# zouyuoz/SVS-UNet-PyTorch

Hardware: AMD Instinct MI355X
Metric: spectrogram-tiles/sec (512x128) U-Net fwd+bwd (L1 train step incl. Adam) (higher is better)
Workload: dtype f32; 1 GPU; train.py L1-loss step, 512x128 tiles, batch 64 per GPU; global_batch=64, parallelism=dp1, mode=train

## Files before the change

### svs_unet_pytorch_amd/csrc/common.h

```cpp
#pragma once
#include <hip/hip_runtime.h>
#include <stdint.h>
#include <stdio.h>
#include <string>
#include <type_traits>

#include "../../include/svs_hip.h"

typedef float f32x4 __attribute__((ext_vector_type(4)));

void svs_set_error(const char* fmt, ...);

#define SVS_REQUIRE(cond, ...)                 \
  do {                                         \
    if (!(cond)) {                             \
      svs_set_error(__VA_ARGS__);              \
      return SVS_ERR_INVALID;                  \
    }                                          \
  } while (0)

#define SVS_CHECK_LAUNCH(name)                                                     \
  do {                                                                             \
    hipError_t e_ = hipGetLastError();                                             \
    if (e_ != hipSuccess) {                                                        \
// ... 4 lines not shown

#define SVS_HIP(call)                                                              \
  do {                                                                             \
    hipError_t e_ = (call);                                                        \
    if (e_ != hipSuccess) {                                                        \
      svs_set_error("%s failed: %s", #call, hipGetErrorString(e_));                \
      return (int)e_;                                                              \
    }                                                                              \
  } while (0)

static inline bool svs_aligned16(const void* p) { return (((uintptr_t)p) & 15u) == 0; }
static inline int svs_cdiv(long a, long b) { return (int)((a + b - 1) / b); }
static inline size_t svs_align_up(size_t x, size_t a) { return (x + a - 1) / a * a; }

enum SvsTune {
  SVS_TUNE_CONV_CFG, SVS_TUNE_CONV_KSPLIT, SVS_TUNE_CONV_WINDOW, SVS_TUNE_CONV_SKIP, SVS_TUNE_SKIP_REDUCE,
  SVS_TUNE_WGRAD_CFG, SVS_TUNE_WGRAD_KSPLIT, SVS_TUNE_WGRAD_SKIP, SVS_TUNE_WGRAD_WINDOW, SVS_TUNE_TRAIN_UNFUSED,
  SVS_TUNE_TRAIN_ONE_STREAM, SVS_TUNE_MFMA_SPLIT, SVS_TUNE_CONV_C1_TILED, SVS_TUNE_BF16_CFG, SVS_TUNE_BF16_KSPLIT,
  SVS_TUNE_BN_INLINE, SVS_TUNE_CONV_GWINDOW, SVS_TUNE_COUNT
};
long svs_tune(int key);
static inline bool svs_tune_on(int key) { return svs_tune(key) >= 0; }
static inline bool svs_tune_flag(int key) { return svs_tune(key) > 0; }

static inline int svs_conv_out(int n) { return (n + 1) / 2; }

__device__ __forceinline__ float svs_wave_sum(float v) {
#pragma unroll
  for (int o = 32; o > 0; o >>= 1) v += __shfl_xor(v, o, 64);
  return v;
}

template <int N_, int I_ = 0, class F>
__device__ __forceinline__ void svs_static_for(F&& f) {
  if constexpr (I_ < N_) {
    f(std::integral_constant<int, I_>{});
    svs_static_for<N_, I_ + 1>(f);
  }
}

template <int R>
__device__ __forceinline__ float svs_quad_bcast(float x) {
  return __builtin_bit_cast(float, __builtin_amdgcn_update_dpp(0, __builtin_bit_cast(int, x), R * 0x55, 0xf, 0xf, true));
}

__device__ __forceinline__ int swz(int row, int chunk) { return chunk ^ ((row >> 1) & 3); }

__host__ __device__ __forceinline__ uint32_t svs_mix32(uint32_t x) {
  x ^= x >> 16; x *= 0x7FEB352Du; x ^= x >> 15; x *= 0x846CA68Bu; x ^= x >> 16;
  return x;
}
__host__ __device__ __forceinline__ uint32_t svs_u32(uint32_t seed, uint64_t idx) {
  uint32_t lo = (uint32_t)idx, hi = (uint32_t)(idx >> 32);
// ... 5 lines not shown
```

### svs_unet_pytorch_amd/csrc/elementwise.hip

```cpp
#include "unet_desc.h"

static inline int red_blocks(long P, int C) {
  long nb = (P * C) / 4096;
  if (nb > 1024) nb = 1024;
  if (nb < 1) nb = 1;
  return (int)nb;
}

struct RedPlan { int sw, nslab, lp, rows; long ppr; };
static RedPlan red_plan(long P, int C) {
  RedPlan r;
  r.sw = C < 32 ? C : 32;
  r.nslab = C / r.sw;
  r.lp = r.sw / 4;
  long nb = (P * C) / 4096;
  if (nb > 512) nb = 512;
  long rows = nb / r.nslab;
  if (rows < 1) rows = 1;
  r.ppr = (P + rows - 1) / rows;
  r.rows = (int)((P + r.ppr - 1) / r.ppr);
  return r;
}
static inline int red_rows(long P, int C) { return red_plan(P, C).rows; }

// ... 230 lines not shown
      if (row == 0) {
        if (dbeta) dbeta[c0 + t] = (float)s;
        if (dgamma) dgamma[c0 + t] = (float)sx;
      }
    }
    __syncthreads();
    k4 = *(const f32x4*)(p.gamma + c) * inv4;
    c1 = *(const f32x4*)&fin[0][l * 4];
    c2 = *(const f32x4*)&fin[1][l * 4];
  } else {
    k4 = *(const f32x4*)(coef + c);
    c1 = *(const f32x4*)(coef + p.C + c);
    c2 = *(const f32x4*)(coef + 2 * p.C + c);
  }
  const long p0 = (long)row * p.ppr;
  long p1 = p0 + p.ppr;
  if (p1 > p.P) p1 = p.P;
  f32x4 acc = {0.f, 0.f, 0.f, 0.f};
#pragma unroll 4
  for (long pix = p0 + pr; pix < p1; pix += PPB) {
    const f32x4 x = *(const f32x4*)(p.raw + pix * p.ldr + c);
    f32x4 dz = *(const f32x4*)(p.dy + pix * p.lddy + c);
    if (p.drop) dz *= *(const f32x4*)(p.drop + (long)((unsigned)pix / (unsigned)p.pps) * p.C + c);
    const f32x4 xm = x - mean4;
    const f32x4 z = xm * k4 + beta4;
#pragma unroll
    for (int k = 0; k < 4; ++k) dz[k] = z[k] > 0.f ? dz[k] : dz[k] * p.slope;
    const f32x4 r = k4 * (dz - c1 - (xm * inv4) * c2);
    *(f32x4*)(d_raw + pix * p.C + c) = r;
    acc += r;
  }
  if (partial) {
    red[t] = acc;
    __syncthreads();
    if (t < p.lp) {
      f32x4 a = red[t];
      for (int j = 1; j < PPB; ++j) a += red[j * p.lp + t];
      *(f32x4*)(partial + (long)row * 2 * p.C + c) = a;
    }
  }
}

static int check_bn(const char* who, const float* raw, long ldr, long P, int C) {
  SVS_REQUIRE(raw, "%s: null pointer", who);
  SVS_REQUIRE(C >= 4 && C % 4 == 0 && C <= 1024 && (256 % (C / 4) == 0 || (C / 4) % 256 == 0), "%s: unsupported C=%d", who, C);
  SVS_REQUIRE(P > 0 && P < (1L << 31) && ldr >= C && ldr % 4 == 0 && svs_aligned16(raw), "%s: bad view", who);
  return SVS_OK;
}

static int grid_for(long total) {
  long g = (total + 255) / 256;
// ... 64 lines not shown
}

extern "C" int svs_bn_act_apply(const float* raw, int64_t ldr, int64_t P, int C, int64_t pixels_per_sample,
                                const float* gamma, const float* beta, const float* save_mean, const float* save_invstd,
                                float slope, const float* drop, float* y, int64_t ldy, hipStream_t stream) {
  int rc = check_bn("svs_bn_act_apply", raw, ldr, P, C);
  if (rc) return rc;
  SVS_REQUIRE(y && ldy >= C && ldy % 4 == 0 && svs_aligned16(y), "svs_bn_act_apply: bad output view");
  BnCtx p{}; p.raw = raw; p.ldr = ldr; p.P = P; p.C = C; p.pps = pixels_per_sample;
  p.gamma = gamma; p.beta = beta; p.mean = save_mean; p.invstd = save_invstd; p.slope = slope; p.drop = drop;
  SVS_REQUIRE(P * (C / 4) < (1L << 32) - 4096L * 256 && pixels_per_sample > 0 && pixels_per_sample < (1L << 31),
              "svs_bn_act_apply: %ld pixels x %d channels need 64-bit indices; split the batch", (long)P, C);
  const int G = C / 4;
  int g_shift = -1;
  if ((G & (G - 1)) == 0) { g_shift = 0; while ((1 << g_shift) < G) ++g_shift; }
  hipLaunchKernelGGL(bn_act_apply_kernel, dim3(grid_for(P * (C / 4))), dim3(256), 0, stream, p, y, (long)ldy, g_shift);
  SVS_CHECK_LAUNCH("bn_act_apply");
  return SVS_OK;
}

int svs_bn_bwd_run(const float* dy, long lddy, const float* raw, long ldr, long P, int C, long pixels_per_sample,
                   const float* gamma, const float* beta, const float* save_mean, const float* save_invstd, float slope,
                   const float* drop, float* d_raw, float* dgamma, float* dbeta, float* dbias, void* ws, size_t ws_bytes,
                   hipStream_t stream, float* dbias_partial, SvsSumJobs* defer);
__global__ void channel_sum_finalize_kernel(const float* __restrict__ partial, int nblk, int C, float* out);

extern "C" int svs_bn_bwd(const float* dy, int64_t lddy, const float* raw, int64_t ldr, int64_t P, int C,
                          int64_t pixels_per_sample, const float* gamma, const float* beta, const float* save_mean,
                          const float* save_invstd, float slope, const float* drop, float* d_raw, float* dgamma,
                          float* dbeta, void* ws, size_t ws_bytes, hipStream_t stream) {
  return svs_bn_bwd_run(dy, lddy, raw, ldr, P, C, pixels_per_sample, gamma, beta, save_mean, save_invstd, slope, drop, d_raw,
                        dgamma, dbeta, nullptr, ws, ws_bytes, stream, nullptr, nullptr);
}

int svs_bn_bwd_run(const float* dy, long lddy, const float* raw, long ldr, long P, int C, long pixels_per_sample,
                   const float* gamma, const float* beta, const float* save_mean, const float* save_invstd, float slope,
                   const float* drop, float* d_raw, float* dgamma, float* dbeta, float* dbias, void* ws, size_t ws_bytes,
                   hipStream_t stream, float* dbias_partial, SvsSumJobs* defer) {
  int rc = check_bn("svs_bn_bwd", raw, ldr, P, C);
  if (rc) return rc;
  SVS_REQUIRE(dy && d_raw && lddy >= C && lddy % 4 == 0 && svs_aligned16(dy) && svs_aligned16(d_raw), "svs_bn_bwd: bad gradient view");
  if (!ws || ws_bytes < svs_bn_workspace_bytes(P, C)) { svs_set_error("svs_bn_bwd: workspace too small"); return SVS_ERR_WORKSPACE; }
  const RedPlan rp = red_plan(P, C);
  const int nb = rp.rows, grid = rp.rows * rp.nslab;
  float* partial = (float*)ws;
  float* coef = partial + (size_t)nb * 2 * C;
  BnCtx p{}; p.raw = raw; p.ldr = ldr; p.P = P; p.C = C; p.pps = pixels_per_sample; set_plan(p, rp);
  p.gamma = gamma; p.beta = beta; p.mean = save_mean; p.invstd = save_invstd; p.slope = slope; p.drop = drop;
  p.dy = dy; p.lddy = lddy;
  hipLaunchKernelGGL(channel_reduce_kernel<1>, dim3(grid), dim3(256), 0, stream, p, partial);
  SVS_CHECK_LAUNCH("bn_bwd_reduce");
  const bool deferred = dbias && dbias_partial && defer && defer->njobs < 12;
  float* bpart = deferred ? dbias_partial : partial;
  if (fin_inline(nb, C) && (!dbias || deferred)) {
    hipLaunchKernelGGL(bn_bwd_apply_kernel<true>, dim3(grid), dim3(256), 0, stream, p, (const float*)nullptr, d_raw, dbias ? bpart : nullptr,
                       (const float*)partial, nb, dgamma, dbeta);
  } else {
    hipLaunchKernelGGL(bn_bwd_finalize_kernel, dim3(C / 4), dim3(256), 0, stream, (const float*)partial, nb, (long)P, C,
                       gamma, save_invstd, dgamma, dbeta, coef);
    SVS_CHECK_LAUNCH("bn_bwd_finalize");
    hipLaunchKernelGGL(bn_bwd_apply_kernel<false>, dim3(grid), dim3(256), 0, stream, p, (const float*)coef, d_raw, dbias ? bpart : nullptr,
                       (const float*)nullptr, 0, (float*)nullptr, (float*)nullptr);
  }
  SVS_CHECK_LAUNCH("bn_bwd_apply");
  if (deferred) {
    const int j = defer->njobs++;
    defer->partial[j] = bpart; defer->nblk[j] = nb; defer->C[j] = C; defer->out[j] = dbias;
  } else if (dbias) {
    hipLaunchKernelGGL(channel_sum_finalize_kernel, dim3(C / 4), dim3(256), 0, stream, (const float*)partial, nb, C, dbias);
    SVS_CHECK_LAUNCH("channel_sum_finalize");
  }
  return SVS_OK;
}

// ... 491 lines not shown
```

### svs_unet_pytorch_amd/csrc/internal.h

```cpp
#pragma once
#include "common.h"

enum { SVS_MODE_GATHER = 0, SVS_MODE_PARITY = 1 };

int svs_conv_gemm_run(int mode, const float* x, long ldx, int B, int H, int W, int C, const float* wp,
                      const float* bias, const float* scale, const float* shift, float slope, float* y, long ldy,
                      int Ho, int Wo, int N, int accumulate, void* ws, size_t ws_bytes, hipStream_t stream,
                      const char* who, float* stats = nullptr, int stats_cap = 0, int* stats_nblk = nullptr);
int svs_bn_finalize_run(const void* partial, int nblk, long P, int C, float eps, float momentum, float* running_mean,
                        float* running_var, long long* nbt, float* save_mean, float* save_invstd, hipStream_t stream);
int svs_bn_fin_act_apply_run(const void* partial, int rows, const float* raw, long ldr, long P, int C, long pixels_per_sample,
                             const float* gamma, const float* beta, float eps, float momentum, float* running_mean,
                             float* running_var, long long* nbt, float* save_mean, float* save_invstd, float slope,
                             const float* drop, float* y, long ldy, hipStream_t stream);
struct SvsSumJobs { int njobs; const float* partial[12]; int nblk[12]; int C[12]; float* out[12]; };
int svs_channel_sum_finalize_multi_run(const SvsSumJobs& jobs, hipStream_t stream);
size_t svs_bn_partial_floats(long P, int C);
int svs_bn_partial_rows(long P, int C);
size_t svs_conv_gemm_workspace(int mode, int B, int H, int W, int C, int Ho, int Wo, int N);

int svs_wgrad_gemm_run(const float* s, long lds, int B, int Hs, int Ws, int Cs, const float* l, long ldl, int Hl,
                       int Wl, int Cl, float* dw, void* ws, size_t ws_bytes, hipStream_t stream, const char* who);
size_t svs_wgrad_gemm_workspace(int B, int Hs, int Ws, int Cs, int Cl);

int svs_conv_c1_run(const float* x, int B, int H, int W, const float* w, const float* bias, const float* scale,
                    const float* shift, float slope, float* y, long ldy, int N, int accumulate, hipStream_t stream,
                    const char* who, long half = 0);
int svs_deconv_to1_run(const float* x, long ldx, int B, int H, int W, int C, const float* w, const float* bias,
                       float* y, int Ho, int Wo, int apply_sigmoid, hipStream_t stream, const char* who, long half = 0);
int svs_wgrad_c1_run(const float* s, long lds, int B, int Hs, int Ws, int Cs, const float* l, int Hl, int Wl,
                     float* dw, void* ws, size_t ws_bytes, hipStream_t stream, const char* who, long half = 0);
size_t svs_wgrad_c1_workspace(int B, int Hs, int Ws, int Cs);

int svs_channel_sum_run(const float* x, long ldx, long P, int C, float* out, void* ws, size_t ws_bytes, hipStream_t stream);
int svs_sum_run(const float* x, long n, float* out, void* ws, size_t ws_bytes, hipStream_t stream);
int svs_eval_loss_acc_run(const float* losses, double alpha_l1, double alpha_mr, double* acc, hipStream_t stream);
int svs_sigmoid_bwd_run(const float* mask, const float* dmask, long n, float* d_logit, hipStream_t stream);

int svs_reduce_slabs_run(const float* slab, int nslab, int per, int groups, long n, float* out, hipStream_t stream);

struct SvsPackJob { const float* w; float* wp; int N, C, kind, first_block; };
struct SvsPackJobs { SvsPackJob j[20]; int n; };
int svs_pack_all_run(SvsPackJobs& jobs, hipStream_t stream);

int svs_bn_bwd_run(const float* dy, long lddy, const float* raw, long ldr, long P, int C, long pixels_per_sample,
                   const float* gamma, const float* beta, const float* save_mean, const float* save_invstd, float slope,
                   const float* drop, float* d_raw, float* dgamma, float* dbeta, float* dbias, void* ws, size_t ws_bytes,
                   hipStream_t stream, float* dbias_partial = nullptr, SvsSumJobs* defer = nullptr);

int svs_fft_twiddles(int n, hipStream_t stream, const float2** out);
int svs_fft_hann(int n, hipStream_t stream, const float** out);

int svs_conv_gemm_describe(int mode, int B, int H, int W, int C, int Ho, int Wo, int N, long ldx, bool inference, char* buf, size_t n);
int svs_wgrad_gemm_describe(int B, int Hs, int Ws, int Cs, int Cl, char* buf, size_t n);
int svs_conv_bf16_describe(int mode, int B, int H, int W, int C, int Ho, int Wo, int N, char* buf, size_t n);
```

### svs_unet_pytorch_amd/csrc/net.hip

```cpp
#include <math.h>
#include <algorithm>
#include <atomic>
#include <mutex>
#include <stdarg.h>
#include <stdlib.h>
#include <string.h>

#include "unet_desc.h"

static thread_local char g_err[512] = "";
void svs_set_error(const char* fmt, ...) {
  va_list ap;
  va_start(ap, fmt);
  vsnprintf(g_err, sizeof(g_err), fmt, ap);
  va_end(ap);
}
extern "C" const char* svs_last_error_string(void) { return g_err; }

static const char* const TUNE_NAMES[SVS_TUNE_COUNT] = {
    "CONV_CFG", "CONV_KSPLIT", "CONV_WINDOW", "CONV_SKIP", "SKIP_REDUCE", "WGRAD_CFG", "WGRAD_KSPLIT", "WGRAD_SKIP",
    "WGRAD_WINDOW", "TRAIN_UNFUSED", "TRAIN_ONE_STREAM", "MFMA_SPLIT", "CONV_C1_TILED", "BF16_CFG", "BF16_KSPLIT", "BN_INLINE",
    "CONV_GWINDOW"};
static std::atomic<long> g_tune[SVS_TUNE_COUNT];
static std::once_flag g_tune_once;
// ... 276 lines not shown
    if ((rc = svs_istft_tiles_n(mix, cs, W, H, 1, mk, 0, mix_phase, 3, B, 2 * H, hop, W, m.wav_pred, nullptr, stream))) return rc;
    if ((rc = svs_istft_tiles_n(voc, cs, W, H, 1, nullptr, 0, voc_phase, 3, B, 2 * H, hop, W, m.wav_tgt, nullptr, stream))) return rc;
    if ((rc = svs_mrstft_loss_fwd_bwd(m.wav_pred, m.wav_tgt, B, L, 0.f, losses + 1, nullptr, m.mr, m.mr_bytes, stream))) return rc;
  } else {
    SVS_HIP(hipMemsetAsync(losses + 1, 0, sizeof(float), stream));
  }
  return acc ? svs_eval_loss_acc_run(losses, alpha_l1, alpha_mr, acc, stream) : SVS_OK;
}

struct TrainWs {
  float* cat[6]; float* c6;
  float* raw[11];
  float* mean[11]; float* invstd[11];
  float* wfwd[12]; float* wbwd[12];
  float* dcat[6]; float* dc6;
  float* d_raw; float* d_logit; float* mask;
  float* d_raw_l[11];
  float* bnws; size_t bnws_bytes;
  float* dbias_part[11];
  float* scratch; size_t scratch_bytes;
  float* scratch2; size_t scratch2_bytes;
  size_t total;
};
#define SVS_FUSED_STATS_ROWS 512
static TrainWs train_layout(const Geo& g, void* ws) {
  TrainWs t{};
  Arena a{(char*)ws, 0};
  auto take = [&](size_t nfloats) { return a.take<float>(nfloats); };
  for (int k = 1; k <= 5; ++k) t.cat[k] = take((size_t)g.P[k] * 2 * CH[k]);
  t.c6 = take((size_t)g.P[6] * CH[6]);
  for (int l = 0; l < 11; ++l) t.raw[l] = take((size_t)g.P[bn_level(l)] * bn_channels(l));
  for (int l = 0; l < 11; ++l) { t.mean[l] = take(bn_channels(l)); t.invstd[l] = take(bn_channels(l)); }
  for (int l = 1; l <= 10; ++l) { t.wfwd[l] = take(param_numel(4 * l)); t.wbwd[l] = take(param_numel(4 * l)); }
  for (int k = 1; k <= 5; ++k) t.dcat[k] = take((size_t)g.P[k] * 2 * CH[k]);
  t.dc6 = take((size_t)g.P[6] * CH[6]);
  size_t dmax = 0;
  for (int k = 1; k <= 6; ++k) if ((size_t)g.P[k] * CH[k] > dmax) dmax = (size_t)g.P[k] * CH[k];
  t.d_raw = take(dmax);
  for (int l = 0; l < 11; ++l) t.d_raw_l[l] = take((size_t)g.P[bn_level(l)] * bn_channels(l));
  t.d_logit = take((size_t)g.P[0]);
  t.mask = take((size_t)g.P[0]);
  size_t bb = 0;
  for (int k = 1; k <= 6; ++k) { size_t s = svs_bn_workspace_bytes(g.P[k], CH[k]); if (s > bb) bb = s; }
  if (bb < (size_t)SVS_FUSED_STATS_ROWS * 2 * CH[6] * sizeof(float)) bb = (size_t)SVS_FUSED_STATS_ROWS * 2 * CH[6] * sizeof(float);
  t.bnws_bytes = bb + 4096;
  t.bnws = take(t.bnws_bytes / sizeof(float));
  for (int l = 0; l < 11; ++l) t.dbias_part[l] = take(svs_bn_partial_floats(g.P[bn_level(l)], bn_channels(l)));
  t.scratch2_bytes = max_layer_bytes(0, 11, [&](const Layer& L) { return bwd_weight_ws(g, L); });
  t.scratch_bytes = std::max({(size_t)4096, t.scratch2_bytes,
                              max_layer_bytes(1, 10, [&](const Layer& L) { return std::max(fwd_ws(g, L), bwd_data_ws(g, L)); })});
  t.scratch = take(t.scratch_bytes / sizeof(float) + 64);
  t.scratch2 = take(t.scratch2_bytes / sizeof(float) + 64);
  t.total = a.used;
  return t;
}

struct SideStream { hipStream_t s; hipEvent_t fork[4], done[4], sync; int nfork; std::mutex mu; };
static SideStream* g_side[64] = {};
static std::mutex g_side_mutex;
static SideStream* side_stream(hipStream_t of) {
  int dev = 0;
  hipDevice_t sdev;
  if (of && hipStreamGetDevice(of, &sdev) == hipSuccess) dev = (int)sdev;
  else if (hipGetDevice(&dev) != hipSuccess) return nullptr;
  if (dev < 0 || dev >= 64) return nullptr;
  std::lock_guard<std::mutex> lock(g_side_mutex);
  if (!g_side[dev]) {
    SideStream* sd = new SideStream();
    int least = 0, greatest = 0;
    bool ok = hipDeviceGetStreamPriorityRange(&least, &greatest) == hipSuccess;
// ... 61 lines not shown
}

static int train_bn_act(const TrainCall& c, int l, int stat_rows, float* bn_buffers, int64_t* nbt, float slope, const float* drop,
                        View y, hipStream_t stream) {
  const TrainWs& t = c.t;
  const int N = bn_channels(l), lvl = bn_level(l);
  const long P = c.g.P[lvl];
  if (!stat_rows) {
    const int rc = svs_bn_stats(t.raw[l], N, P, N, t.bnws, t.bnws_bytes, stream);
    if (rc) return rc;
    stat_rows = svs_bn_partial_rows(P, N);
  }
  return svs_bn_fin_act_apply_run(t.bnws, stat_rows, t.raw[l], N, P, N, (long)c.g.h[lvl] * c.g.w[lvl], c.v.gamma[l], c.v.beta[l], BN_EPS,
                                  BN_MOMENTUM, bn_buffers ? bn_buffers + svs_unet_buffer_offset(l, 0) : nullptr,
                                  bn_buffers ? bn_buffers + svs_unet_buffer_offset(l, 1) : nullptr,
                                  nbt ? (long long*)(nbt + l) : nullptr, t.mean[l], t.invstd[l], slope, drop, y.p, y.ld, stream);
}

static int train_forward_impl(const TrainCall& c, float* bn_buffers, int64_t* nbt, const float* mix, const float* drop, float* mask,
                              hipStream_t stream) {
  const Geo& g = c.g; const TrainWs& t = c.t; const ParamView& v = c.v;
  const int B = g.B;
  int rc;
  const int fused_rows = svs_tune_flag(SVS_TUNE_TRAIN_UNFUSED) ? 0 : (int)(t.bnws_bytes / sizeof(float));
  SideStream* sd = svs_tune_flag(SVS_TUNE_TRAIN_ONE_STREAM) ? nullptr : side_stream(stream);
  std::unique_lock<std::mutex> guard;
  if (sd) guard = std::unique_lock<std::mutex>(sd->mu);
  {
    SvsPackJobs jobs{};
    for (int l = 1; l <= 10; ++l) {
      const Layer& L = LAYERS[l];
      jobs.j[jobs.n++] = SvsPackJob{v.w[l], t.wfwd[l], L.N, L.C, L.up, 0};
      jobs.j[jobs.n++] = SvsPackJob{v.w[l], t.wbwd[l], L.C, L.N, !L.up, 0};
    }
    if (sd) {
      SVS_HIP(hipEventRecord(sd->fork[0], stream));
      SVS_HIP(hipStreamWaitEvent(sd->s, sd->fork[0], 0));
    }
    if ((rc = svs_pack_all_run(jobs, sd ? sd->s : stream))) return rc;
    if (sd) SVS_HIP(hipEventRecord(sd->done[0], sd->s));
  }
  for (int k = 1; k <= 6; ++k) {
    if (k == 2 && sd) SVS_HIP(hipStreamWaitEvent(stream, sd->done[0], 0));
    const int l = k - 1;
    const View xi = (k == 1) ? View{const_cast<float*>(mix), 1} : cat_half(t.cat, g, k - 1, 1);
    int stat_rows = 0;
    if (k == 1) rc = svs_enc_block_fwd(xi.p, xi.ld, B, g.h[0], g.w[0], 1, v.w[0], v.b[0], nullptr, nullptr, 0.f, t.raw[0], CH[1], CH[1], 0,
// ... 7 lines not shown
  }
  const float* dp = drop;
  for (int l = 6; l <= 10; ++l) {
    const Layer& D = LAYERS[l];
    const float* x = (l == 6) ? t.c6 : t.cat[D.lin];
    int stat_rows = 0;
    rc = svs_conv_gemm_run(SVS_MODE_PARITY, x, D.C, B, g.h[D.lin], g.w[D.lin], D.C, t.wfwd[l], v.b[l], nullptr, nullptr, 0.f,
                           t.raw[l], D.N, g.h[D.lout], g.w[D.lout], D.N, 0, t.scratch, t.scratch_bytes, stream,
                           "deconv forward", t.bnws, fused_rows, &stat_rows);
    if (rc) return rc;
    if ((rc = train_bn_act(c, l, stat_rows, bn_buffers, nbt, 0.f, dp, cat_half(t.cat, g, D.lout, 0), stream))) return rc;
    if (dp) dp += (long)B * D.N;
  }
  return svs_deconv_to1_run(t.cat[1], CH[1], B, g.h[1], g.w[1], LAYERS[11].C, v.w[11], v.b[11], mask, g.h[0], g.w[0], 1, stream,
                            "svs_unet_train_forward", level1_plane(g));
}

static int train_backward_impl(const TrainCall& c, float* grads, const float* mix, const float* drop, hipStream_t stream, int parts = 15) {
  const Geo& g = c.g; const TrainWs& t = c.t; const ParamView& v = c.v;
  const int B = g.B;
  int rc;
  auto G = [&](int idx) { return grads + svs_unet_param_offset(idx); };
  SvsSumJobs sums{};
  const bool unfused = svs_tune_flag(SVS_TUNE_TRAIN_UNFUSED);
  SideStream* sd = svs_tune_flag(SVS_TUNE_TRAIN_ONE_STREAM) ? nullptr : side_stream(stream);
  std::unique_lock<std::mutex> guard;
  if (sd) guard = std::unique_lock<std::mutex>(sd->mu);
  const hipStream_t wstream = sd ? sd->s : stream;
  float* const wscratch = sd ? t.scratch2 : t.scratch;
  const size_t wscratch_bytes = sd ? t.scratch2_bytes : t.scratch_bytes;
  int nfork_local = 0;
  int& nfork = sd ? sd->nfork : nfork_local;
  if (parts & 1) nfork = 0;
  auto layer_draw = [&](int l) -> float* { return sd ? t.d_raw_l[l] : t.d_raw; };
  auto fork = [&]() -> int {
    if (!sd) return SVS_OK;
    SVS_HIP(hipEventRecord(sd->fork[nfork & 3], stream));
    SVS_HIP(hipStreamWaitEvent(sd->s, sd->fork[nfork & 3], 0));
    return SVS_OK;
  };
  auto forked = [&]() -> int { ++nfork; return SVS_OK; };
  auto join = [&]() -> int {
    if (sd && nfork > 0) {
      SVS_HIP(hipEventRecord(sd->done[0], sd->s));
      SVS_HIP(hipStreamWaitEvent(stream, sd->done[0], 0));
    }
    return SVS_OK;
// ... 15 lines not shown
    const View dyv = cat_half(t.dcat, g, lout, 0);
    float* const d_raw = layer_draw(l);
    rc = svs_bn_bwd_run(dyv.p, dyv.ld, t.raw[l], N, g.P[lout], N, (long)g.h[lout] * g.w[lout], v.gamma[l], v.beta[l],
                        t.mean[l], t.invstd[l], 0.f, drop ? drop + drop_off[l] : nullptr, d_raw, G(4 * l + 2), G(4 * l + 3),
                        G(4 * l + 1), t.bnws, t.bnws_bytes, stream, unfused ? nullptr : t.dbias_part[l], &sums);
    if (rc) return rc;
    if ((rc = fork())) return rc;
    if ((rc = svs_dec_block_bwd_weight(x, C, B, g.h[lin], g.w[lin], C, d_raw, N, g.h[lout], g.w[lout], N, G(4 * l), nullptr,
                                       wscratch, wscratch_bytes, wstream))) return rc;
    if ((rc = forked())) return rc;
    float* dx = (l == 6) ? t.dc6 : t.dcat[lin];
    if ((rc = svs_dec_block_bwd_data(d_raw, N, B, g.h[lout], g.w[lout], N, t.wbwd[l], dx, C, g.h[lin], g.w[lin], C, 0,
                                     t.scratch, t.scratch_bytes, stream))) return rc;
  }
  if ((rc = svs_channel_sum_finalize_multi_run(sums, stream))) return rc;
  sums.njobs = 0;
  }
  if (!(parts & 14)) return SVS_OK;
  for (int k = 6; k >= 1; --k) {
    if (!(parts & (k == 6 ? 2 : k >= 4 ? 4 : 8))) continue;
    const int l = k - 1, N = CH[k], C = CH[k - 1];
    const View dyv = (k == 6) ? View{t.dc6, CH[6]} : cat_half(t.dcat, g, k, 1);
    float* const d_raw = layer_draw(l);
    rc = svs_bn_bwd_run(dyv.p, dyv.ld, t.raw[l], N, g.P[k], N, (long)g.h[k] * g.w[k], v.gamma[l], v.beta[l], t.mean[l], t.invstd[l],
                        LEAKY, nullptr, d_raw, G(4 * l + 2), G(4 * l + 3), G(4 * l + 1), t.bnws, t.bnws_bytes, stream,
                        unfused ? nullptr : t.dbias_part[l], &sums);
    if (rc) return rc;
    const View xi = (k == 1) ? View{const_cast<float*>(mix), 1} : cat_half(t.cat, g, k - 1, 1);
    const float* x = xi.p; const long ldx = xi.ld;
    if (k == 1) {
      if ((rc = svs_enc_block_bwd_weight(d_raw, N, B, g.h[k], g.w[k], N, x, ldx, g.h[k - 1], g.w[k - 1], C, G(4 * l), nullptr,
                                         t.scratch, t.scratch_bytes, stream))) return rc;
      continue;
    }
    if ((rc = fork())) return rc;
    if ((rc = svs_enc_block_bwd_weight(d_raw, N, B, g.h[k], g.w[k], N, x, ldx, g.h[k - 1], g.w[k - 1], C, G(4 * l), nullptr,
                                       wscratch, wscratch_bytes, wstream))) return rc;
    if ((rc = forked())) return rc;
    if (k >= 2) {
      const View dxs = cat_half(t.dcat, g, k - 1, 1);
      if ((rc = svs_enc_block_bwd_data(d_raw, N, B, g.h[k], g.w[k], N, t.wbwd[l], dxs.p, dxs.ld, g.h[k - 1], g.w[k - 1], C, 1,
                                       t.scratch, t.scratch_bytes, stream))) return rc;
    }
  }
  if ((rc = svs_channel_sum_finalize_multi_run(sums, stream))) return rc;
  return (parts & 8) ? join() : SVS_OK;
}

extern "C" int svs_unet_train_bwd_sync(hipStream_t consumer) {
  SideStream* sd = svs_tune_flag(SVS_TUNE_TRAIN_ONE_STREAM) ? nullptr : side_stream(consumer);
  if (!sd) return SVS_OK;
  std::lock_guard<std::mutex> guard(sd->mu);
// ... 117 lines not shown
```

### svs_unet_pytorch_amd/csrc/special.hip

```cpp
#include "internal.h"

struct C1Args {
  const float* x; int B, H, W;
  const float* w;
  const float* bias; const float* scale; const float* shift; float slope;
  float* y; long ldy; int Ho, Wo; int accumulate;
  long half;
};

__device__ __forceinline__ long chan_off(long pix, long ld, int sub, int subs_per_half, long half) {
  return pix * ld + (half ? (sub >= subs_per_half ? half + (sub - subs_per_half) * 4 : sub * 4) : sub * 4);
}

template <int COUT>
__global__ __launch_bounds__(256) void conv_c1_kernel(C1Args p) {
  constexpr int G = COUT / 4;
  constexpr int LD = COUT + 4;
  __shared__ __attribute__((aligned(16))) float tile[256 * LD];
  const float* __restrict__ w = p.w;
  const long P = (long)p.B * p.Ho * p.Wo;
  const long pix0 = (long)blockIdx.x * 256;
  const long pix = pix0 + threadIdx.x;
  if (pix < P) {
    const unsigned upix = (unsigned)pix, utmp = upix / (unsigned)p.Wo;
// ... 323 lines not shown
    }
  }
#pragma unroll
  for (int k = 0; k < 25; ++k)
#pragma unroll
    for (int c = 0; c < 4; ++c) {
      float v = acc[k][c];
#pragma unroll
      for (int s = G; s < 64; s <<= 1) v += __shfl_xor(v, s, 64);
      acc[k][c] = v;
    }
  const int lane = t & 63, wave = t >> 6;
  if (lane < G) {
#pragma unroll
    for (int k = 0; k < 25; ++k)
#pragma unroll
      for (int c = 0; c < 4; ++c) red[wave][(lane * 4 + c) * 25 + k] = acc[k][c];
  }
  __syncthreads();
  float* out = p.slab + (long)blockIdx.x * (25 * CS);
  for (int i = t; i < 25 * CS; i += 256) out[i] = (red[0][i] + red[1][i]) + (red[2][i] + red[3][i]);
}

template <int CS>
__global__ __launch_bounds__(256) void wgrad_c1_mfma_kernel(WgC1Args p, int ntiles, int tiles_per_wave) {
  constexpr int TH = 4, TW = 16, MT = CS / 16;
  constexpr int LS = (CS == 32) ? 48 : 16;
  constexpr int LH = 2 * TH + 3, LW = 2 * TW + 3, LWP = LW + 1;
  constexpr int NSP = TH * TW * (CS / 4) / 64;
  constexpr int NLP = (LH * LW + 63) / 64;
  __shared__ __attribute__((aligned(16))) float Ssm[4][TH * TW * LS];
  __shared__ float Lsm[4][LH * LWP];
  const int t = threadIdx.x, lane = t & 63, wave = t >> 6;
  const int lrow = lane & 15, q = lane >> 4;
  float* const sS = Ssm[wave];
  float* const sL = Lsm[wave];
  const int tiles_w = (p.Ws + TW - 1) / TW, tiles_h = (p.Hs + TH - 1) / TH;
  const int gw = blockIdx.x * 4 + wave;
  const int tile_lo = gw * tiles_per_wave;
  const int tile_hi = min(tile_lo + tiles_per_wave, ntiles);

  f32x4 sreg[NSP];
  float lreg[NLP];
  auto fetch = [&](int tile) {
    const int tw0 = (tile % tiles_w) * TW, th0 = ((tile / tiles_w) % tiles_h) * TH;
    const long b = tile / (tiles_w * tiles_h);
#pragma unroll
    for (int r = 0; r < NSP; ++r) {
      const int e = lane + 64 * r;
      const int c4 = e % (CS / 4), px = e / (CS / 4);
      const int sh = th0 + px / TW, sw = tw0 + px % TW;
      f32x4 v = {0.f, 0.f, 0.f, 0.f};
      if (sh < p.Hs && sw < p.Ws) v = *(const f32x4*)(p.s + chan_off((b * p.Hs + sh) * p.Ws + sw, p.lds, c4, CS / 8, p.half));
      sreg[r] = v;
    }
    const float* img = p.l + b * p.Hl * p.Wl;
#pragma unroll
    for (int r = 0; r < NLP; ++r) {
      const int e = lane + 64 * r;
      const int wr = e / LW, wc = e % LW;
      const int ih = 2 * th0 - 2 + wr, iw = 2 * tw0 - 2 + wc;
      float v = 0.f;
      if (e < LH * LW && (unsigned)ih < (unsigned)p.Hl && (unsigned)iw < (unsigned)p.Wl) v = img[(long)ih * p.Wl + iw];
      lreg[r] = v;
    }
  };
  auto stage = [&]() {
#pragma unroll
    for (int r = 0; r < NSP; ++r) {
      const int e = lane + 64 * r;
      *(f32x4*)(&sS[(e / (CS / 4)) * LS + (e % (CS / 4)) * 4]) = sreg[r];
    }
#pragma unroll
    for (int r = 0; r < NLP; ++r) {
      const int e = lane + 64 * r;
      if (e < LH * LW) sL[(e / LW) * LWP + e % LW] = lreg[r];
    }
  };
  f32x4 acc[MT][2];
#pragma unroll
  for (int i = 0; i < MT; ++i) { acc[i][0] = (f32x4){0.f, 0.f, 0.f, 0.f}; acc[i][1] = acc[i][0]; }
  int boff[2];
#pragma unroll
  for (int nt = 0; nt < 2; ++nt) {
    const int tap = min(nt * 16 + lrow, 24);
    boff[nt] = (tap / 5) * LWP + tap % 5 + 2 * q;
  }
  if (tile_lo < tile_hi) fetch(tile_lo);
  for (int tile = tile_lo; tile < tile_hi; ++tile) {
    stage();
    if (tile + 1 < tile_hi) fetch(tile + 1);
#pragma unroll
    for (int ks = 0; ks < TH * TW / 4; ++ks) {
      const int sh = ks / 4, sg = ks % 4;
      float bv[2];
#pragma unroll
      for (int nt = 0; nt < 2; ++nt) bv[nt] = sL[boff[nt] + 2 * sh * LWP + 8 * sg];
#pragma unroll
      for (int i = 0; i < MT; ++i) {
        const float a = sS[(sh * TW + sg * 4 + q) * LS + i * 16 + lrow];
#pragma unroll
        for (int nt = 0; nt < 2; ++nt) acc[i][nt] = __builtin_amdgcn_mfma_f32_16x16x4f32(a, bv[nt], acc[i][nt], 0, 0, 0);
      }
    }
  }
  float* out = p.slab + (long)gw * (25 * CS);
#pragma unroll
  for (int i = 0; i < MT; ++i)
#pragma unroll
    for (int nt = 0; nt < 2; ++nt) {
      const int tap = nt * 16 + lrow;
      if (tap < 25) {
#pragma unroll
        for (int r = 0; r < 4; ++r) out[(i * 16 + 4 * q + r) * 25 + tap] = acc[i][nt][r];
      }
    }
}

__global__ __launch_bounds__(256) void reduce_slabs_kernel(const float* __restrict__ slab, int nslab, int per, long n,
                                                           float* __restrict__ out) {
  const long i = ((long)blockIdx.x * 256 + threadIdx.x) * 4;
  if (i >= n) return;
  const int z0 = blockIdx.y * per;
  int z1 = z0 + per;
  if (z1 > nslab) z1 = nslab;
  const float* src = slab + (long)z0 * n + i;
  f32x4 s = {0.f, 0.f, 0.f, 0.f};
  int z = z0;
  for (; z + 4 <= z1; z += 4, src += 4 * n) {
    const f32x4 a = *(const f32x4*)src, b = *(const f32x4*)(src + n), c = *(const f32x4*)(src + 2 * n), d = *(const f32x4*)(src + 3 * n);
    s += a; s += b; s += c; s += d;
  }
  for (; z < z1; ++z, src += n) s += *(const f32x4*)src;
  *(f32x4*)(out + (long)blockIdx.y * n + i) = s;
}

int svs_reduce_slabs_run(const float* slab, int nslab, int per, int groups, long n, float* out, hipStream_t stream) {
  hipLaunchKernelGGL(reduce_slabs_kernel, dim3((unsigned)((n / 4 + 255) / 256), (unsigned)groups), dim3(256), 0, stream, slab, nslab, per, n, out);
  SVS_CHECK_LAUNCH("reduce_slabs");
  return SVS_OK;
}

#define C1_GROUPS 32

static int wgrad_c1_blocks(long P) {
  long nb = (P + 2047) / 2048;
  if (nb > 1024) nb = 1024;
  if (nb < 1) nb = 1;
  return (int)nb;
}

size_t svs_wgrad_c1_workspace(int B, int Hs, int Ws, int Cs) {
  (void)B; (void)Hs; (void)Ws;
  return (size_t)(1024 + C1_GROUPS) * 25 * Cs * sizeof(float);
}

int svs_wgrad_c1_run(const float* s, long lds, int B, int Hs, int Ws, int Cs, const float* l, int Hl, int Wl,
                     float* dw, void* ws, size_t ws_bytes, hipStream_t stream, const char* who, long half) {
  SVS_REQUIRE(s && l && dw, "%s: null pointer", who);
  SVS_REQUIRE(Cs == 16 || Cs == 32, "%s: supports Cs=16/32, got %d", who, Cs);
  SVS_REQUIRE(Hs == svs_conv_out(Hl) && Ws == svs_conv_out(Wl), "%s: grid mismatch", who);
  SVS_REQUIRE(lds >= (half ? Cs / 2 : Cs) && lds % 4 == 0 && svs_aligned16(s), "%s: bad view", who);
  const long P = (long)B * Hs * Ws;
  const int nb = wgrad_c1_blocks(P);
  const size_t need = svs_wgrad_c1_workspace(B, Hs, Ws, Cs);
  if (!ws || ws_bytes < need) {
    svs_set_error("%s: workspace too small (%zu < %zu)", who, ws_bytes, need);
    return SVS_ERR_WORKSPACE;
  }
  WgC1Args a{s, lds, B, Hs, Ws, l, Hl, Wl, (float*)ws, (P + nb - 1) / nb, half};
  int nslab = nb;
  const int ntiles = B * ((Hs + 3) / 4) * ((Ws + 15) / 16);
  if (ntiles >= 256) {
    int waves = ntiles < 1024 ? ntiles : 1024;
    waves = (waves + 3) / 4 * 4;
    if (waves > 1024) waves = 1024;
    const int tpw = (ntiles + waves - 1) / waves;
    waves = ((ntiles + tpw - 1) / tpw + 3) / 4 * 4;
    nslab = waves;
    if (Cs == 16) hipLaunchKernelGGL(wgrad_c1_mfma_kernel<16>, dim3(waves / 4), dim3(256), 0, stream, a, ntiles, tpw);
    else hipLaunchKernelGGL(wgrad_c1_mfma_kernel<32>, dim3(waves / 4), dim3(256), 0, stream, a, ntiles, tpw);
  } else if (Cs == 16) hipLaunchKernelGGL(wgrad_c1_kernel<16>, dim3(nb), dim3(256), 0, stream, a);
  else hipLaunchKernelGGL(wgrad_c1_kernel<32>, dim3(nb), dim3(256), 0, stream, a);
  SVS_CHECK_LAUNCH("wgrad_c1");
  const long n = 25L * Cs;
  float* tmp = (float*)ws + (size_t)nslab * n;
  const int groups = nslab < C1_GROUPS ? nslab : C1_GROUPS;
  const int per = (nslab + groups - 1) / groups;
  const unsigned gx = (unsigned)((n / 4 + 255) / 256);
  hipLaunchKernelGGL(reduce_slabs_kernel, dim3(gx, (unsigned)groups), dim3(256), 0, stream, (const float*)ws, nslab, per, n, tmp);
  SVS_CHECK_LAUNCH("reduce_slabs");
  hipLaunchKernelGGL(reduce_slabs_kernel, dim3(gx, 1), dim3(256), 0, stream, (const float*)tmp, groups, groups, n, dw);
  SVS_CHECK_LAUNCH("reduce_slabs");
  return SVS_OK;
}
```

Baseline: 20140 tiles/s.

## Fuse conv1 BatchNorm backward apply into the first-layer weight-gradient MFMA kernel

For the first encoder layer, BN backward now only runs its reduction and finalize to produce coefficients. The BN/leaky-ReLU gradient is then recomputed on the fly inside the conv1 weight-gradient MFMA kernel, which also emits per-wave bias-gradient partials for the deferred sum. This avoids writing and re-reading the d_raw tensor for the largest-resolution layer and drops one elementwise pass. The cost is extra register pressure in the wgrad kernel and a larger dbias partial buffer.

Result: no change. 20330 tiles/s, median of 6 (+1.0%).

```diff
diff --git a/svs_unet_pytorch_amd/csrc/common.h b/svs_unet_pytorch_amd/csrc/common.h
--- a/svs_unet_pytorch_amd/csrc/common.h
+++ b/svs_unet_pytorch_amd/csrc/common.h
@@ -50,6 +50,8 @@
 long svs_tune(int key);
 static inline bool svs_tune_on(int key) { return svs_tune(key) >= 0; }
 static inline bool svs_tune_flag(int key) { return svs_tune(key) > 0; }
+static inline bool svs_unfused_all() { const long v = svs_tune(SVS_TUNE_TRAIN_UNFUSED); return v > 0 && v != 2; }
+static inline bool svs_unfused_conv1_bwd() { return svs_tune(SVS_TUNE_TRAIN_UNFUSED) > 0; }
 
 static inline int svs_conv_out(int n) { return (n + 1) / 2; }
 
@@ -57,6 +59,14 @@
 #pragma unroll
   for (int o = 32; o > 0; o >>= 1) v += __shfl_xor(v, o, 64);
   return v;
+}
+
+__device__ __forceinline__ f32x4 svs_bn_bwd_term(f32x4 x, f32x4 dz, f32x4 mean4, f32x4 inv4, f32x4 k4, f32x4 beta4, f32x4 c1, f32x4 c2, float slope) {
+  const f32x4 xm = x - mean4;
+  const f32x4 z = xm * k4 + beta4;
+#pragma unroll
+  for (int k = 0; k < 4; ++k) dz[k] = z[k] > 0.f ? dz[k] : dz[k] * slope;
+  return k4 * (dz - c1 - (xm * inv4) * c2);
 }
 
 template <int N_, int I_ = 0, class F>
diff --git a/svs_unet_pytorch_amd/csrc/elementwise.hip b/svs_unet_pytorch_amd/csrc/elementwise.hip
--- a/svs_unet_pytorch_amd/csrc/elementwise.hip
+++ b/svs_unet_pytorch_amd/csrc/elementwise.hip
@@ -276,11 +276,7 @@
     const f32x4 x = *(const f32x4*)(p.raw + pix * p.ldr + c);
     f32x4 dz = *(const f32x4*)(p.dy + pix * p.lddy + c);
     if (p.drop) dz *= *(const f32x4*)(p.drop + (long)((unsigned)pix / (unsigned)p.pps) * p.C + c);
-    const f32x4 xm = x - mean4;
-    const f32x4 z = xm * k4 + beta4;
-#pragma unroll
-    for (int k = 0; k < 4; ++k) dz[k] = z[k] > 0.f ? dz[k] : dz[k] * p.slope;
-    const f32x4 r = k4 * (dz - c1 - (xm * inv4) * c2);
+    const f32x4 r = svs_bn_bwd_term(x, dz, mean4, inv4, k4, beta4, c1, c2, p.slope);
     *(f32x4*)(d_raw + pix * p.C + c) = r;
     acc += r;
   }
@@ -391,7 +387,7 @@
 int svs_bn_bwd_run(const float* dy, long lddy, const float* raw, long ldr, long P, int C, long pixels_per_sample,
                    const float* gamma, const float* beta, const float* save_mean, const float* save_invstd, float slope,
                    const float* drop, float* d_raw, float* dgamma, float* dbeta, float* dbias, void* ws, size_t ws_bytes,
-                   hipStream_t stream, float* dbias_partial, SvsSumJobs* defer);
+                   hipStream_t stream, float* dbias_partial, SvsSumJobs* defer, const float** coef_out);
 __global__ void channel_sum_finalize_kernel(const float* __restrict__ partial, int nblk, int C, float* out);
 
 extern "C" int svs_bn_bwd(const float* dy, int64_t lddy, const float* raw, int64_t ldr, int64_t P, int C,
@@ -399,16 +395,16 @@
                           const float* save_invstd, float slope, const float* drop, float* d_raw, float* dgamma,
                           float* dbeta, void* ws, size_t ws_bytes, hipStream_t stream) {
   return svs_bn_bwd_run(dy, lddy, raw, ldr, P, C, pixels_per_sample, gamma, beta, save_mean, save_invstd, slope, drop, d_raw,
-                        dgamma, dbeta, nullptr, ws, ws_bytes, stream, nullptr, nullptr);
+                        dgamma, dbeta, nullptr, ws, ws_bytes, stream, nullptr, nullptr, nullptr);
 }
 
 int svs_bn_bwd_run(const float* dy, long lddy, const float* raw, long ldr, long P, int C, long pixels_per_sample,
                    const float* gamma, const float* beta, const float* save_mean, const float* save_invstd, float slope,
                    const float* drop, float* d_raw, float* dgamma, float* dbeta, float* dbias, void* ws, size_t ws_bytes,
-                   hipStream_t stream, float* dbias_partial, SvsSumJobs* defer) {
+                   hipStream_t stream, float* dbias_partial, SvsSumJobs* defer, const float** coef_out) {
   int rc = check_bn("svs_bn_bwd", raw, ldr, P, C);
   if (rc) return rc;
-  SVS_REQUIRE(dy && d_raw && lddy >= C && lddy % 4 == 0 && svs_aligned16(dy) && svs_aligned16(d_raw), "svs_bn_bwd: bad gradient view");
+  SVS_REQUIRE(dy && (d_raw || coef_out) && lddy >= C && lddy % 4 == 0 && svs_aligned16(dy) && svs_aligned16(d_raw), "svs_bn_bwd: bad gradient view");
   if (!ws || ws_bytes < svs_bn_workspace_bytes(P, C)) { svs_set_error("svs_bn_bwd: workspace too small"); return SVS_ERR_WORKSPACE; }
   const RedPlan rp = red_plan(P, C);
   const int nb = rp.rows, grid = rp.rows * rp.nslab;
@@ -419,6 +415,13 @@
   p.dy = dy; p.lddy = lddy;
   hipLaunchKernelGGL(channel_reduce_kernel<1>, dim3(grid), dim3(256), 0, stream, p, partial);
   SVS_CHECK_LAUNCH("bn_bwd_reduce");
+  if (coef_out) {
+    hipLaunchKernelGGL(bn_bwd_finalize_kernel, dim3(C / 4), dim3(256), 0, stream, (const float*)partial, nb, (long)P, C,
+                       gamma, save_invstd, dgamma, dbeta, coef);
+    SVS_CHECK_LAUNCH("bn_bwd_finalize");
+    *coef_out = coef;
+    return SVS_OK;
+  }
   const bool deferred = dbias && dbias_partial && defer && defer->njobs < 12;
   float* bpart = deferred ? dbias_partial : partial;
   if (fin_inline(nb, C) && (!dbias || deferred)) {
diff --git a/svs_unet_pytorch_amd/csrc/internal.h b/svs_unet_pytorch_amd/csrc/internal.h
--- a/svs_unet_pytorch_amd/csrc/internal.h
+++ b/svs_unet_pytorch_amd/csrc/internal.h
@@ -29,7 +29,14 @@
 int svs_deconv_to1_run(const float* x, long ldx, int B, int H, int W, int C, const float* w, const float* bias,
                        float* y, int Ho, int Wo, int apply_sigmoid, hipStream_t stream, const char* who, long half = 0);
 int svs_wgrad_c1_run(const float* s, long lds, int B, int Hs, int Ws, int Cs, const float* l, int Hl, int Wl,
-                     float* dw, void* ws, size_t ws_bytes, hipStream_t stream, const char* who, long half = 0);
+                     float* dw, void* ws, size_t ws_bytes, hipStream_t stream, const char* who, long half = 0,
+                     const struct SvsWgradBn* bn = nullptr);
+struct SvsWgradBn {
+  const float* dy; long lddy; const float* raw; long ldr;
+  const float* coef; const float* mean; const float* invstd; const float* beta; float slope;
+  float* dbias_partial; size_t dbias_cap;
+};
+int svs_wgrad_c1_bn_rows(int B, int Hs, int Ws, int Cs);
 size_t svs_wgrad_c1_workspace(int B, int Hs, int Ws, int Cs);
 
 int svs_channel_sum_run(const float* x, long ldx, long P, int C, float* out, void* ws, size_t ws_bytes, hipStream_t stream);
@@ -46,7 +53,7 @@
 int svs_bn_bwd_run(const float* dy, long lddy, const float* raw, long ldr, long P, int C, long pixels_per_sample,
                    const float* gamma, const float* beta, const float* save_mean, const float* save_invstd, float slope,
                    const float* drop, float* d_raw, float* dgamma, float* dbeta, float* dbias, void* ws, size_t ws_bytes,
-                   hipStream_t stream, float* dbias_partial = nullptr, SvsSumJobs* defer = nullptr);
+                   hipStream_t stream, float* dbias_partial = nullptr, SvsSumJobs* defer = nullptr, const float** coef_out = nullptr);
 
 int svs_fft_twiddles(int n, hipStream_t stream, const float2** out);
 int svs_fft_hann(int n, hipStream_t stream, const float** out);
diff --git a/svs_unet_pytorch_amd/csrc/net.hip b/svs_unet_pytorch_amd/csrc/net.hip
--- a/svs_unet_pytorch_amd/csrc/net.hip
+++ b/svs_unet_pytorch_amd/csrc/net.hip
@@ -322,6 +322,11 @@
   float* scratch2; size_t scratch2_bytes;
   size_t total;
 };
+static size_t dbias_part_floats(const Geo& g, int l) {
+  size_t n = svs_bn_partial_floats(g.P[bn_level(l)], bn_channels(l));
+  if (l == 0) n = std::max(n, (size_t)svs_wgrad_c1_bn_rows(g.B, g.h[1], g.w[1], CH[1]) * 2 * CH[1]);
+  return n;
+}
 #define SVS_FUSED_STATS_ROWS 512
 static TrainWs train_layout(const Geo& g, void* ws) {
   TrainWs t{};
@@ -345,7 +350,7 @@
   if (bb < (size_t)SVS_FUSED_STATS_ROWS * 2 * CH[6] * sizeof(float)) bb = (size_t)SVS_FUSED_STATS_ROWS * 2 * CH[6] * sizeof(float);
   t.bnws_bytes = bb + 4096;
   t.bnws = take(t.bnws_bytes / sizeof(float));
-  for (int l = 0; l < 11; ++l) t.dbias_part[l] = take(svs_bn_partial_floats(g.P[bn_level(l)], bn_channels(l)));
+  for (int l = 0; l < 11; ++l) t.dbias_part[l] = take(dbias_part_floats(g, l));
   t.scratch2_bytes = max_layer_bytes(0, 11, [&](const Layer& L) { return bwd_weight_ws(g, L); });
   t.scratch_bytes = std::max({(size_t)4096, t.scratch2_bytes,
                               max_layer_bytes(1, 10, [&](const Layer& L) { return std::max(fwd_ws(g, L), bwd_data_ws(g, L)); })});
@@ -453,7 +458,7 @@
   const Geo& g = c.g; const TrainWs& t = c.t; const ParamView& v = c.v;
   const int B = g.B;
   int rc;
-  const int fused_rows = svs_tune_flag(SVS_TUNE_TRAIN_UNFUSED) ? 0 : (int)(t.bnws_bytes / sizeof(float));
+  const int fused_rows = svs_unfused_all() ? 0 : (int)(t.bnws_bytes / sizeof(float));
   SideStream* sd = svs_tune_flag(SVS_TUNE_TRAIN_ONE_STREAM) ? nullptr : side_stream(stream);
   std::unique_lock<std::mutex> guard;
   if (sd) guard = std::unique_lock<std::mutex>(sd->mu);
@@ -507,7 +512,7 @@
   int rc;
   auto G = [&](int idx) { return grads + svs_unet_param_offset(idx); };
   SvsSumJobs sums{};
-  const bool unfused = svs_tune_flag(SVS_TUNE_TRAIN_UNFUSED);
+  const bool unfused = svs_unfused_all();
   SideStream* sd = svs_tune_flag(SVS_TUNE_TRAIN_ONE_STREAM) ? nullptr : side_stream(stream);
   std::unique_lock<std::mutex> guard;
   if (sd) guard = std::unique_lock<std::mutex>(sd->mu);
@@ -569,12 +574,25 @@
     const int l = k - 1, N = CH[k], C = CH[k - 1];
     const View dyv = (k == 6) ? View{t.dc6, CH[6]} : cat_half(t.dcat, g, k, 1);
     float* const d_raw = layer_draw(l);
+    const View xi = (k == 1) ? View{const_cast<float*>(mix), 1} : cat_half(t.cat, g, k - 1, 1);
+    const float* x = xi.p; const long ldx = xi.ld;
+    const int c1_rows = (k == 1 && !svs_unfused_conv1_bwd()) ? svs_wgrad_c1_bn_rows(B, g.h[1], g.w[1], N) : 0;
+    if (c1_rows > 0 && (size_t)c1_rows * 2 * N <= dbias_part_floats(g, l) && sums.njobs < 12) {
+      const float* coef = nullptr;
+      rc = svs_bn_bwd_run(dyv.p, dyv.ld, t.raw[l], N, g.P[k], N, (long)g.h[k] * g.w[k], v.gamma[l], v.beta[l], t.mean[l], t.invstd[l],
+                          LEAKY, nullptr, nullptr, G(4 * l + 2), G(4 * l + 3), nullptr, t.bnws, t.bnws_bytes, stream, nullptr, nullptr, &coef);
+      if (rc) return rc;
+      const SvsWgradBn bn{dyv.p, dyv.ld, t.raw[l], N, coef, t.mean[l], t.invstd[l], v.beta[l], LEAKY, t.dbias_part[l], dbias_part_floats(g, l)};
+      if ((rc = svs_wgrad_c1_run(nullptr, N, B, g.h[k], g.w[k], N, x, g.h[k - 1], g.w[k - 1], G(4 * l), t.scratch, t.scratch_bytes, stream,
+                                 "conv1 bwd_weight", 0, &bn))) return rc;
+      const int j = sums.njobs++;
+      sums.partial[j] = t.dbias_part[l]; sums.nblk[j] = c1_rows; sums.C[j] = N; sums.out[j] = G(4 * l + 1);
+      continue;
+    }
     rc = svs_bn_bwd_run(dyv.p, dyv.ld, t.raw[l], N, g.P[k], N, (long)g.h[k] * g.w[k], v.gamma[l], v.beta[l], t.mean[l], t.invstd[l],
                         LEAKY, nullptr, d_raw, G(4 * l + 2), G(4 * l + 3), G(4 * l + 1), t.bnws, t.bnws_bytes, stream,
                         unfused ? nullptr : t.dbias_part[l], &sums);
     if (rc) return rc;
-    const View xi = (k == 1) ? View{const_cast<float*>(mix), 1} : cat_half(t.cat, g, k - 1, 1);
-    const float* x = xi.p; const long ldx = xi.ld;
     if (k == 1) {
       if ((rc = svs_enc_block_bwd_weight(d_raw, N, B, g.h[k], g.w[k], N, x, ldx, g.h[k - 1], g.w[k - 1], C, G(4 * l), nullptr,
                                          t.scratch, t.scratch_bytes, stream))) return rc;
diff --git a/svs_unet_pytorch_amd/csrc/special.hip b/svs_unet_pytorch_amd/csrc/special.hip
--- a/svs_unet_pytorch_amd/csrc/special.hip
+++ b/svs_unet_pytorch_amd/csrc/special.hip
@@ -369,8 +369,14 @@
   for (int i = t; i < 25 * CS; i += 256) out[i] = (red[0][i] + red[1][i]) + (red[2][i] + red[3][i]);
 }
 
-template <int CS>
-__global__ __launch_bounds__(256) void wgrad_c1_mfma_kernel(WgC1Args p, int ntiles, int tiles_per_wave) {
+struct WgC1Bn {
+  const float* dy; long lddy; const float* raw; long ldr;
+  const float* coef; const float* mean; const float* invstd; const float* beta; float slope;
+  float* dbias_partial;
+};
+
+template <int CS, bool BN>
+__device__ __forceinline__ void wgrad_c1_mfma_body(const WgC1Args& p, const WgC1Bn& n, int ntiles, int tiles_per_wave) {
   constexpr int TH = 4, TW = 16, MT = CS / 16;
   constexpr int LS = (CS == 32) ? 48 : 16;
   constexpr int LH = 2 * TH + 3, LW = 2 * TW + 3, LWP = LW + 1;
@@ -389,16 +395,36 @@
 
   f32x4 sreg[NSP];
   float lreg[NLP];
+  f32x4 xreg[BN ? NSP : 1], bsum = {0.f, 0.f, 0.f, 0.f}, mean4, inv4, k4, beta4, c1, c2;
+  unsigned live = 0;
+  if constexpr (BN) {
+    static_assert(64 % (CS / 4) == 0, "a lane keeps one channel group");
+    const int c = (lane % (CS / 4)) * 4;
+    mean4 = *(const f32x4*)(n.mean + c); inv4 = *(const f32x4*)(n.invstd + c); beta4 = *(const f32x4*)(n.beta + c);
+    k4 = *(const f32x4*)(n.coef + c); c1 = *(const f32x4*)(n.coef + CS + c); c2 = *(const f32x4*)(n.coef + 2 * CS + c);
+  }
   auto fetch = [&](int tile) {
     const int tw0 = (tile % tiles_w) * TW, th0 = ((tile / tiles_w) % tiles_h) * TH;
     const long b = tile / (tiles_w * tiles_h);
+    if constexpr (BN) live = 0;
 #pragma unroll
     for (int r = 0; r < NSP; ++r) {
       const int e = lane + 64 * r;
       const int c4 = e % (CS / 4), px = e / (CS / 4);
       const int sh = th0 + px / TW, sw = tw0 + px % TW;
       f32x4 v = {0.f, 0.f, 0.f, 0.f};
-      if (sh < p.Hs && sw < p.Ws) v = *(const f32x4*)(p.s + chan_off((b * p.Hs + sh) * p.Ws + sw, p.lds, c4, CS / 8, p.half));
+      if constexpr (BN) {
+        f32x4 x = v;
+        if (sh < p.Hs && sw < p.Ws) {
+          const long pix = (b * p.Hs + sh) * p.Ws + sw;
+          v = *(const f32x4*)(n.dy + pix * n.lddy + c4 * 4);
+          x = *(const f32x4*)(n.raw + pix * n.ldr + c4 * 4);
+          live |= 1u << r;
+        }
+        xreg[r] = x;
+      } else {
+        if (sh < p.Hs && sw < p.Ws) v = *(const f32x4*)(p.s + chan_off((b * p.Hs + sh) * p.Ws + sw, p.lds, c4, CS / 8, p.half));
+      }
       sreg[r] = v;
     }
     const float* img = p.l + b * p.Hl * p.Wl;
@@ -416,6 +442,11 @@
 #pragma unroll
     for (int r = 0; r < NSP; ++r) {
       const int e = lane + 64 * r;
+      if constexpr (BN) {
+        const f32x4 d = svs_bn_bwd_term(xreg[r], sreg[r], mean4, inv4, k4, beta4, c1, c2, n.slope);
+        sreg[r] = (live >> r & 1u) ? d : (f32x4){0.f, 0.f, 0.f, 0.f};
+        bsum += sreg[r];
+      }
       *(f32x4*)(&sS[(e / (CS / 4)) * LS + (e % (CS / 4)) * 4]) = sreg[r];
     }
 #pragma unroll
@@ -462,6 +493,26 @@
         for (int r = 0; r < 4; ++r) out[(i * 16 + 4 * q + r) * 25 + tap] = acc[i][nt][r];
       }
     }
+  if constexpr (BN) {
+#pragma unroll
+    for (int k = 0; k < 4; ++k)
+#pragma unroll
+      for (int o = CS / 4; o < 64; o <<= 1) bsum[k] += __shfl_xor(bsum[k], o, 64);
+    if (lane < CS / 4) {
+      float* row = n.dbias_partial + (long)gw * (2 * CS) + lane * 4;
+      *(f32x4*)row = bsum;
+      *(f32x4*)(row + CS) = (f32x4){0.f, 0.f, 0.f, 0.f};
+    }
+  }
+}
+
+template <int CS>
+__global__ __launch_bounds__(256) void wgrad_c1_mfma_kernel(WgC1Args p, int ntiles, int tiles_per_wave) {
+  wgrad_c1_mfma_body<CS, false>(p, WgC1Bn{}, ntiles, tiles_per_wave);
+}
+template <int CS>
+__global__ __launch_bounds__(256) void wgrad_c1_mfma_bn_kernel(WgC1Args p, WgC1Bn n, int ntiles, int tiles_per_wave) {
+  wgrad_c1_mfma_body<CS, true>(p, n, ntiles, tiles_per_wave);
 }
 
 __global__ __launch_bounds__(256) void reduce_slabs_kernel(const float* __restrict__ slab, int nslab, int per, long n,
@@ -502,12 +553,25 @@
   return (size_t)(1024 + C1_GROUPS) * 25 * Cs * sizeof(float);
 }
 
+struct WgC1Plan { int ntiles, waves, tpw; };
+static WgC1Plan wgrad_c1_plan(int B, int Hs, int Ws) {
+  WgC1Plan w{B * ((Hs + 3) / 4) * ((Ws + 15) / 16), 0, 0};
+  if (w.ntiles < 256) return w;
+  int waves = w.ntiles < 1024 ? w.ntiles : 1024;
+  waves = (waves + 3) / 4 * 4;
+  if (waves > 1024) waves = 1024;
+  w.tpw = (w.ntiles + waves - 1) / waves;
+  w.waves = ((w.ntiles + w.tpw - 1) / w.tpw + 3) / 4 * 4;
+  return w;
+}
+int svs_wgrad_c1_bn_rows(int B, int Hs, int Ws, int Cs) { return Cs == 16 ? wgrad_c1_plan(B, Hs, Ws).waves : 0; }
+
 int svs_wgrad_c1_run(const float* s, long lds, int B, int Hs, int Ws, int Cs, const float* l, int Hl, int Wl,
-                     float* dw, void* ws, size_t ws_bytes, hipStream_t stream, const char* who, long half) {
-  SVS_REQUIRE(s && l && dw, "%s: null pointer", who);
+                     float* dw, void* ws, size_t ws_bytes, hipStream_t stream, const char* who, long half, const SvsWgradBn* bn) {
+  SVS_REQUIRE((s || bn) && l && dw, "%s: null pointer", who);
   SVS_REQUIRE(Cs == 16 || Cs == 32, "%s: supports Cs=16/32, got %d", who, Cs);
   SVS_REQUIRE(Hs == svs_conv_out(Hl) && Ws == svs_conv_out(Wl), "%s: grid mismatch", who);
-  SVS_REQUIRE(lds >= (half ? Cs / 2 : Cs) && lds % 4 == 0 && svs_aligned16(s), "%s: bad view", who);
+  SVS_REQUIRE(bn || (lds >= (half ? Cs / 2 : Cs) && lds % 4 == 0 && svs_aligned16(s)), "%s: bad view", who);
   const long P = (long)B * Hs * Ws;
   const int nb = wgrad_c1_blocks(P);
   const size_t need = svs_wgrad_c1_workspace(B, Hs, Ws, Cs);
@@ -517,13 +581,18 @@
   }
   WgC1Args a{s, lds, B, Hs, Ws, l, Hl, Wl, (float*)ws, (P + nb - 1) / nb, half};
   int nslab = nb;
-  const int ntiles = B * ((Hs + 3) / 4) * ((Ws + 15) / 16);
-  if (ntiles >= 256) {
-    int waves = ntiles < 1024 ? ntiles : 1024;
-    waves = (waves + 3) / 4 * 4;
-    if (waves > 1024) waves = 1024;
-    const int tpw = (ntiles + waves - 1) / waves;
-    waves = ((ntiles + tpw - 1) / tpw + 3) / 4 * 4;
+  const WgC1Plan wp = wgrad_c1_plan(B, Hs, Ws);
+  const int ntiles = wp.ntiles, waves = wp.waves, tpw = wp.tpw;
+  if (bn) {
+    SVS_REQUIRE(waves > 0 && Cs == 16 && (size_t)waves * 2 * Cs <= bn->dbias_cap, "%s: the fused BatchNorm backward needs the MFMA form, 16 channels "
+                "and %d bias-gradient rows", who, waves);
+    SVS_REQUIRE(bn->dy && bn->raw && bn->coef && bn->mean && bn->invstd && bn->beta && bn->dbias_partial && bn->lddy >= Cs && bn->lddy % 4 == 0 &&
+                bn->ldr >= Cs && bn->ldr % 4 == 0 && svs_aligned16(bn->dy) && svs_aligned16(bn->raw) && svs_aligned16(bn->dbias_partial),
+                "%s: bad BatchNorm-backward descriptor", who);
+    const WgC1Bn n{bn->dy, bn->lddy, bn->raw, bn->ldr, bn->coef, bn->mean, bn->invstd, bn->beta, bn->slope, bn->dbias_partial};
+    nslab = waves;
+    hipLaunchKernelGGL(wgrad_c1_mfma_bn_kernel<16>, dim3(waves / 4), dim3(256), 0, stream, a, n, ntiles, tpw);
+  } else if (waves > 0) {
     nslab = waves;
     if (Cs == 16) hipLaunchKernelGGL(wgrad_c1_mfma_kernel<16>, dim3(waves / 4), dim3(256), 0, stream, a, ntiles, tpw);
     else hipLaunchKernelGGL(wgrad_c1_mfma_kernel<32>, dim3(waves / 4), dim3(256), 0, stream, a, ntiles, tpw);
```
